# Gadersd/stable-diffusion-burn

Measured on NVIDIA H100. Metric: images_per_sec_512x512_20steps, higher is better.
Workload: dtype fp16 tensor-core operands (3-term split-fp16 on the two high-res UNet levels), fp32 accumulate

## Files before the change

stable_diffusion_burn_b200/csrc/api.cu:

```cuda
#include "../../include/sdb200.h"

#include <dlfcn.h>

#include <cstdlib>
#include <cstring>
#include <mutex>

#include "attention.cuh"
#include "kernels.cuh"
#include "model.cuh"
#include "runtime.cuh"

using namespace sdb;

struct sdb_ctx {
  Ctx c;
};

static thread_local std::string g_err;

#define API_BEGIN(ctxp)                      \
  if (!(ctxp)) {                             \
    g_err = "null context";                  \
    return 1;                                \
// ... 305 lines not shown
  API_BEGIN(ctx)
  need_final(c);
  model_sample_dev(c, d_context, n, L, d_uncond, Lu, guidance_scale, n_steps, d_init_latent, H, W, nullptr, d_rgb,
                   (cudaStream_t)stream);
  API_END
}

int sdb_forward_diffuser(sdb_ctx* ctx, const float* latent, int32_t timestep, const float* context, int n, int L,
                         const float* uncond, int Lu, double guidance_scale, int H, int W, float* pred, float* out_uncond,
                         float* out_cond) {
  API_BEGIN(ctx)
  need_final(c);
  SDB_CHECK(latent && context && uncond, "null argument");
  model_forward_diffuser_host(c, latent, timestep, context, n, L, uncond, Lu, guidance_scale, H, W, pred, out_uncond, out_cond);
  API_END
}

int sdb_forward_diffuser_dev(sdb_ctx* ctx, const float* d_latent, int32_t timestep, const float* d_context, int n, int L,
                             const float* d_uncond, int Lu, double guidance_scale, int H, int W, float* d_pred, void* stream) {
  API_BEGIN(ctx)
  need_final(c);
  model_forward_diffuser_dev(c, d_latent, timestep, d_context, n, L, d_uncond, Lu, guidance_scale, H, W, d_pred, nullptr, nullptr,
                             (cudaStream_t)stream);
  API_END
}

int sdb_encode_image(sdb_ctx* ctx, const float* img, int n, int H, int W, float* latent) {
  API_BEGIN(ctx)
  need_final(c);
  SDB_CHECK(img && latent, "null argument");
  model_encode_host(c, img, n, H, W, latent);
  API_END
}

int sdb_encode_image_dev(sdb_ctx* ctx, const float* d_img, int n, int H, int W, float* d_latent, void* stream) {
  API_BEGIN(ctx)
  need_final(c);
  model_encode_dev(c, d_img, n, H, W, d_latent, (cudaStream_t)stream);
  API_END
}

int sdb_clip_forward(sdb_ctx* ctx, const int32_t* tokens, int n, int L, float* out) {
  API_BEGIN(ctx)
  need_final(c);
  SDB_CHECK(tokens && out, "null argument");
  model_clip_forward_host(c, tokens, n, L, out);
  API_END
}

int sdb_clip_forward_dev(sdb_ctx* ctx, const int32_t* d_tokens, int n, int L, float* d_out, void* stream) {
  API_BEGIN(ctx)
  need_final(c);
  model_clip_forward_dev(c, d_tokens, n, L, d_out, (cudaStream_t)stream);
  API_END
}

int sdb_set_option(sdb_ctx* ctx, const char* key, int value) {
  API_BEGIN(ctx)
  const std::string k = key ? key : "";
  if (k == "precision")
    c.opt_precision = value;
  else if (k == "graphs")
    c.opt_graphs = value;
  else if (k == "splitk")
    c.opt_splitk = value;
  else if (k == "raw16")
    c.opt_raw16 = value;
  else if (k == "splitk_min_iters")
    c.opt_splitk_min_iters = value;
  else if (k == "splitk_chunk")
    c.opt_splitk_chunk = value < 1 ? 1 : value;
  else if (k == "attn_split")
    c.opt_attn_split = value;
  else if (k == "attn_regsplit")
    g_attn_regsplit = value;
  else if (k == "emb_hoist")
    c.opt_emb_hoist = value;
  else if (k == "prefetch_w")
    c.opt_prefetch_w = value;
  else if (k == "mlp_passes")
    c.opt_mlp_passes = value;
  else if (k == "gn_epilogue")
    c.opt_gn_epilogue = value;
  else if (k == "skip_merge")
    c.opt_skip_merge = value;
  else if (k == "gn_apply_ctas")
    g_gn_apply_ctas = value < 1 ? 1 : value;
  else if (k == "gn_min_pix")
    g_gn_min_pix = value < 1 ? 1 : value;
  else
    throw Error("unknown option: " + k);
  model_invalidate_graphs(c);
  API_END
}

int sdb_profile_enable(sdb_ctx* ctx, int on) {
  API_BEGIN(ctx)
  profile_collect(c);
  c.profiling = on != 0;
  API_END
}
int sdb_profile_reset(sdb_ctx* ctx) {
  API_BEGIN(ctx)
  profile_collect(c);
  c.launches = 0;
  for (int i = 0; i < KC_COUNT; ++i) c.cls_ms[i] = c.cls_flops[i] = c.cls_bytes[i] = c.cls_issued[i] = 0, c.cls_launches[i] = 0;
  API_END
}
int sdb_profile_class_count(sdb_ctx*) { return KC_COUNT; }
int sdb_profile_get(sdb_ctx* ctx, int cls, const char** name, int64_t* launches, double* ms, double* flops, double* bytes) {
  API_BEGIN(ctx)
  SDB_CHECK(cls >= 0 && cls < KC_COUNT, "class index");
  profile_collect(c);
  if (name) *name = kernel_class_name(cls);
  if (launches) *launches = c.cls_launches[cls];
  if (ms) *ms = c.cls_ms[cls];
  if (flops) *flops = c.cls_flops[cls];
  if (bytes) *bytes = c.cls_bytes[cls];
  API_END
}
int sdb_profile_get_issued(sdb_ctx* ctx, int cls, double* issued_flops) {
  API_BEGIN(ctx)
  SDB_CHECK(cls >= 0 && cls < KC_COUNT && issued_flops, "class index");
  *issued_flops = c.cls_issued[cls];
  API_END
}
int64_t sdb_launch_count(sdb_ctx* ctx) { return ctx ? ctx->c.launches : -1; }

int sdb_test_linear(sdb_ctx* ctx, const float* a, const float* w, const float* bias, int M, int K, int N, int passes,
                    float* out) {
  API_BEGIN(ctx)
  c.work.reset();
  float* d_a = c.work.get<float>((size_t)M * K);
  float* d_w = c.work.get<float>((size_t)K * N);
  float* d_b = bias ? c.work.get<float>(N) : nullptr;
  float* d_c = c.work.get<float>((size_t)M * N);
  SDB_CUDA(cudaMemcpyAsync(d_a, a, sizeof(float) * M * K, cudaMemcpyHostToDevice, c.stream));
  SDB_CUDA(cudaMemcpyAsync(d_w, w, sizeof(float) * K * N, cudaMemcpyHostToDevice, c.stream));
  if (bias) SDB_CUDA(cudaMemcpyAsync(d_b, bias, sizeof(float) * N, cudaMemcpyHostToDevice, c.stream));
  ActOp A;
  A.p.hi = c.work.get<__half>((size_t)M * K);
  A.p.lo = c.work.get<__half>((size_t)M * K);
  A.W = M, A.C = K;
  WeightOp Wp;
  Wp.p.hi = c.work.get<__half>((size_t)N * K);
  Wp.p.lo = c.work.get<__half>((size_t)N * K);
  Wp.N = N, Wp.K = K;
  convert_f16_launch(d_a, (long long)M * K, A.p, c.stream);
  pack_linear_launch(d_w, K, N, Wp.p, 0, c.stream);
  Epilogue ep;
  ep.out_f32 = d_c;
  ep.bias = d_b;
  run_gemm(c, G_LINEAR, A, nullptr, Wp, passes, ep);
  SDB_CUDA(cudaMemcpyAsync(out, d_c, sizeof(float) * M * N, cudaMemcpyDeviceToHost, c.stream));
  SDB_CUDA(cudaStreamSynchronize(c.stream));
  API_END
}

int sdb_test_gemm_ex(sdb_ctx* ctx, const float* a, const float* w, const float* bias, const float* residual, int M, int K, int N,
                     int passes, int flags, const float* xa, const float* xw, int XK, float* out) {
  API_BEGIN(ctx)
  c.work.reset();
  const bool geglu = flags & 1, from_f16 = flags & 4;
  SDB_CHECK(!geglu || (N % 128 == 0 && !residual && !xa), "GEGLU test: N (= 2 * hidden) must be a multiple of 128, no residual / extra K");
  const int Nout = geglu ? N / 2 : N;
  auto up = [&](const float* h, size_t cnt) {
// ... 319 lines not shown
```

stable_diffusion_burn_b200/csrc/gemm_tc.cu:

```cuda
#include "gemm_tc.cuh"

#include <cstring>

namespace sdb {

static constexpr int BM = 128;
static constexpr int BK = 64;
static constexpr int A_TILE_BYTES = BM * BK * 2;

template <int BN, int PASSES>
struct StageLayout {
  static constexpr int B_TILE_BYTES = BN * BK * 2;
  static constexpr int A_TILES = PASSES >= 2 ? 2 : 1;
  static constexpr int B_TILES = PASSES >= 3 ? 2 : 1;
  static constexpr int BYTES = A_TILES * A_TILE_BYTES + B_TILES * B_TILE_BYTES;
};
template <int BN>
struct AccLayout {
  static constexpr int PITCH = (BN + 4) * 4;
  static constexpr int BYTES = BM * PITCH;
  static constexpr int GN_BYTES = 32 * 1024;
};
static constexpr int EW = 8;

__device__ __noinline__ void epilogue_store(float4 f, unsigned int o32, unsigned int o16, float* out_f32, __half* out_f16,
                                            __half* out_f16_lo, int act) {
  if (act == 1) {
    f.x = __fdividef(f.x, 1.0f + __expf(-1.702f * f.x)), f.y = __fdividef(f.y, 1.0f + __expf(-1.702f * f.y));
    f.z = __fdividef(f.z, 1.0f + __expf(-1.702f * f.z)), f.w = __fdividef(f.w, 1.0f + __expf(-1.702f * f.w));
  }
  if (out_f32) *reinterpret_cast<float4*>(out_f32 + o32) = f;
  if (out_f16) {
    __half2 h[2] = {f2h2_sat(f.x, f.y), f2h2_sat(f.z, f.w)};
    *reinterpret_cast<uint2*>(out_f16 + o16) = *reinterpret_cast<uint2*>(h);
    if (out_f16_lo) {
      const float2 f0 = __half22float2(h[0]), f1 = __half22float2(h[1]);
      __half2 l[2] = {__floats2half2_rn(f.x - f0.x, f.y - f0.y), __floats2half2_rn(f.z - f1.x, f.w - f1.y)};
      *reinterpret_cast<uint2*>(out_f16_lo + o16) = *reinterpret_cast<uint2*>(l);
    }
  }
}

struct GnTile {
  int tn, img0, tile, nimg;
};
__device__ __forceinline__ GnTile gn_tile_of(const GemmParams& p, int n0, int th, int tw) {
  GnTile g;
  if (p.gn_rpi) {
    g.nimg = p.gn_nimg;
    if (p.gn_rpi >= BM)
      g.tn = 1, g.img0 = (tw * BM) / p.gn_rpi, g.tile = ((tw * BM) % p.gn_rpi) / BM;
    else
      g.tn = BM / p.gn_rpi, g.img0 = tw * g.tn, g.tile = 0;
  } else {
    g.tn = p.TN, g.img0 = n0, g.tile = th * p.tiles_w + tw, g.nimg = p.nimg;
  }
  return g;
}
__device__ __forceinline__ void gn_write_partials(const GemmParams& p, const float2* cs, int BN, int te, int nthreads, const GnTile g,
                                                  int col0, int z) {
  const int nbk_tile = BN / p.gn_bucket, nbk_total = p.N / p.gn_bucket;
  const int qpi = 4 / g.tn;
  const int slot = p.gn_slot0 + g.tile * p.split_k + z;
  (void)nthreads;
  if (te < ((nbk_tile * 4 + 31) & ~31)) {
    const int b = te >> 2, q = te & 3;
    float sm = 0.f, sq = 0.f;
    if (b < nbk_tile) {
      const float2* src = cs + q * BN + b * p.gn_bucket;
      for (int c = 0; c < p.gn_bucket; ++c) sm += src[c].x, sq += src[c].y;
    }
    if (qpi >= 2) sm += __shfl_xor_sync(0xffffffffu, sm, 1), sq += __shfl_xor_sync(0xffffffffu, sq, 1);
    if (qpi == 4) sm += __shfl_xor_sync(0xffffffffu, sm, 2), sq += __shfl_xor_sync(0xffffffffu, sq, 2);
    const int k = q / qpi, img = g.img0 + k, c0 = b * p.gn_bucket;
    if (b < nbk_tile && (q % qpi) == 0 && img < g.nimg && col0 + c0 < p.N) {
      float2* dst = reinterpret_cast<float2*>(p.gn_part) + ((size_t)img * p.gn_cap + slot) * nbk_total + (col0 + c0) / p.gn_bucket;
      *dst = make_float2(sm, sq);
    }
  }
}

enum : int { EPI_PLAIN = 0, EPI_GN = 1, EPI_LNS = 2, EPI_LNC = 3, EPI_GEGLU = 4, EPI_GEGLU_LNC = 5 };

template <int BN, int PASSES, int STAGES>
// ... 427 lines not shown
#pragma unroll
            for (int b4 = 0; b4 < 2; ++b4) {
              float4 t[4];
#pragma unroll
              for (int i = 0; i < 4; ++i)
                asm volatile("ld.shared.v4.f32 {%0, %1, %2, %3}, [%4];"
                             : "=f"(t[i].x), "=f"(t[i].y), "=f"(t[i].z), "=f"(t[i].w)
                             : "r"(tl + (b4 * 4 + i) * 4 * TROW)
                             : "memory");
#pragma unroll
              for (int i = 0; i < 4; ++i) {
                const int k = b4 * 4 + i;
                if (mr8[k] < 0) continue;
                float4 f = t[i];
                if constexpr (kLNC) {
                  f.x = rs8[k] * (f.x - mu8[k] * us[j].x), f.y = rs8[k] * (f.y - mu8[k] * us[j].y);
                  f.z = rs8[k] * (f.z - mu8[k] * us[j].z), f.w = rs8[k] * (f.w - mu8[k] * us[j].w);
                }
                if constexpr (kLNC)
                  f.x += bvs[j].x, f.y += bvs[j].y, f.z += bvs[j].z, f.w += bvs[j].w;
                else
                  f.x += bvs[j].x + ad[k].x, f.y += bvs[j].y + ad[k].y, f.z += bvs[j].z + ad[k].z, f.w += bvs[j].w + ad[k].w;
                if constexpr (kLNS) {
                  lrs[k] += (f.x + f.y) + (f.z + f.w);
                  lrq[k] = fmaf(f.x, f.x, fmaf(f.y, f.y, fmaf(f.z, f.z, fmaf(f.w, f.w, lrq[k]))));
                }
                if constexpr (kGN) {
                  gsum.x += f.x, gsum.y += f.y, gsum.z += f.z, gsum.w += f.w;
                  gsq.x = fmaf(f.x, f.x, gsq.x), gsq.y = fmaf(f.y, f.y, gsq.y), gsq.z = fmaf(f.z, f.z, gsq.z), gsq.w = fmaf(f.w, f.w, gsq.w);
                }
                epilogue_store(f, (unsigned)(mr8[k] * p.ldc + col), (unsigned)(mr8[k] * p.ldc16 + col), p.out_f32, p.out_f16,
                               p.out_f16_lo, p.act);
              }
            }
          }
          if constexpr (kGN) {
#pragma unroll
            for (int o = 8; o <= 16; o <<= 1) {
              gsum.x += __shfl_xor_sync(0xffffffffu, gsum.x, o), gsum.y += __shfl_xor_sync(0xffffffffu, gsum.y, o);
              gsum.z += __shfl_xor_sync(0xffffffffu, gsum.z, o), gsum.w += __shfl_xor_sync(0xffffffffu, gsum.w, o);
              gsq.x += __shfl_xor_sync(0xffffffffu, gsq.x, o), gsq.y += __shfl_xor_sync(0xffffffffu, gsq.y, o);
              gsq.z += __shfl_xor_sync(0xffffffffu, gsq.z, o), gsq.w += __shfl_xor_sync(0xffffffffu, gsq.w, o);
            }
            if (sub == 0) {
              float2* d = gn_cs + q * BN + c + cq;
              d[0] = make_float2(gsum.x, gsq.x), d[1] = make_float2(gsum.y, gsq.y);
              d[2] = make_float2(gsum.z, gsq.z), d[3] = make_float2(gsum.w, gsq.w);
            }
          }
          if (j + 1 < NCH && c + CSTEP < BN) issue_addends(col0 + c + CSTEP + cq);
        }
      }
      if constexpr (kLNS) {
#pragma unroll
        for (int k = 0; k < 8; ++k) {
#pragma unroll
          for (int o = 1; o <= 4; o <<= 1) {
            lrs[k] += __shfl_xor_sync(0xffffffffu, lrs[k], o);
            lrq[k] += __shfl_xor_sync(0xffffffffu, lrq[k], o);
          }
        }
        if ((lane & 7) == 0) {
          const int slot = blockIdx.y * 2 + half;
#pragma unroll
          for (int k = 0; k < 8; ++k)
            if (mr8[k] >= 0) {
              float2* d = reinterpret_cast<float2*>(p.ln_out) + (size_t)mr8[k] * p.ln_slots + slot;
              d[0] = make_float2(lrs[k], lrq[k]);
              if (EG == 1) d[1] = make_float2(0.f, 0.f);
            }
        }
      }
      if constexpr (kGN) {
        asm volatile("bar.sync 1, %0;" ::"n"(EW * 32) : "memory");
        gn_write_partials(p, gn_cs, BN, threadIdx.x - 128, EW * 32, gnt, col0, p.up2 ? (int)blockIdx.z * p.gn_phase_slots : 0);
      }
    }
    if (dbg && threadIdx.x == 128) dbg[6] = clock64();
  }
  __syncthreads();
  if (dbg && threadIdx.x == 0) dbg[7] = clock64();
}

static constexpr int SMEM_OPTIN_MAX = 227 * 1024;
template <int BN, int PASSES>
constexpr int pick_stages() {
  constexpr int per = StageLayout<BN, PASSES>::BYTES;
  constexpr int n = (SMEM_OPTIN_MAX - 1024) / (per + 2 * 8);
  return n > 8 ? 8 : n;
}

template <int BN, int PASSES, int STAGES, int EPI>
static void launch_epi(const GemmMaps& maps, const GemmParams& p, cudaStream_t stream) {
  constexpr int smem = region_bytes<BN, PASSES, STAGES>() + 2 * STAGES * 8 + 1024;
  static_assert(smem <= SMEM_OPTIN_MAX, "shared memory per block");
  static_assert(4 * BN * 8 <= AccLayout<BN>::GN_BYTES && 2 * (EW * 32) * 4 * 16 <= AccLayout<BN>::GN_BYTES,
                "GroupNorm column sums must fit in the scratch after the accumulator image");
  static DeviceOnce once;
  if (once.first())
    SDB_CUDA(cudaFuncSetAttribute(gemm_tc_kernel<BN, PASSES, STAGES, EPI>, cudaFuncAttributeMaxDynamicSharedMemorySize, smem));
  dim3 grid(p.tiles_n * p.tiles_h * p.tiles_w, (p.N + BN - 1) / BN, p.up2 ? 4 : p.split_k);
  launch_k(gemm_tc_kernel<BN, PASSES, STAGES, EPI>, grid, dim3(128 + 32 * EW), (size_t)smem, stream, maps, p);
}
template <int BN, int PASSES, int STAGES>
static void launch_inst(const GemmMaps& maps, const GemmParams& p, cudaStream_t stream) {
  SDB_CHECK((p.gn_part != nullptr) + (p.ln_out != nullptr) + (p.ln_in != nullptr) <= 1, "one statistics role per launch");
  if constexpr (BN == 128) {
    if (p.geglu) {
      SDB_CHECK(!p.gn_part && !p.ln_out && p.split_k == 1, "GEGLU epilogue: no statistics output, no split-K");
      return p.ln_in ? launch_epi<BN, PASSES, STAGES, EPI_GEGLU_LNC>(maps, p, stream)
                     : launch_epi<BN, PASSES, STAGES, EPI_GEGLU>(maps, p, stream);
    }
  }
  SDB_CHECK(!p.geglu, "the GEGLU epilogue is built for 128-wide tiles");
  if constexpr (BN >= 128) {
    if (p.gn_part) return launch_epi<BN, PASSES, STAGES, EPI_GN>(maps, p, stream);
  }
  if constexpr (BN == 160) {
    if (p.ln_out) return launch_epi<BN, PASSES, STAGES, EPI_LNS>(maps, p, stream);
  }
  if constexpr (BN == 128 || BN == 160) {
    if (p.ln_in) return launch_epi<BN, PASSES, STAGES, EPI_LNC>(maps, p, stream);
  }
  SDB_CHECK(!p.gn_part && !p.ln_out && !p.ln_in, "this statistics epilogue is not built for this tile width");
  launch_epi<BN, PASSES, STAGES, EPI_PLAIN>(maps, p, stream);
}
bool gemm_tc_supports(int BN, int epi) {
  return epi == EPI_PLAIN || (epi == EPI_GN && BN >= 128) || (epi == EPI_LNS && BN == 160) || (epi == EPI_LNC && (BN == 128 || BN == 160));
}

template <int BN, int PASSES>
static void launch_bn(const GemmMaps& maps, const GemmParams& p, cudaStream_t stream) {
  launch_inst<BN, PASSES, pick_stages<BN, PASSES>()>(maps, p, stream);
}

void gemm_tc_launch(const GemmMaps& maps, const GemmParams& p, int BN, int passes, cudaStream_t stream) {
  SDB_CHECK(p.TN * p.TH * p.TW == BM, "M tile must cover 128 rows");
  SDB_CHECK(p.N % 32 == 0, "N must be a multiple of 32");
#define SDB_DISPATCH(bn)                                             \
  case bn:                                                           \
    if (passes == 1) launch_bn<bn, 1>(maps, p, stream);              \
    else if (passes == 2) launch_bn<bn, 2>(maps, p, stream);         \
    else launch_bn<bn, 3>(maps, p, stream);                          \
    break;
  switch (BN) {
    SDB_DISPATCH(64)
    SDB_DISPATCH(128)
    SDB_DISPATCH(160)
    SDB_DISPATCH(256)
    default:
      throw Error("unsupported BN");
  }
#undef SDB_DISPATCH
}

}
```

stable_diffusion_burn_b200/csrc/gemm_tc.cuh:

```cuda
#pragma once
#include "common.cuh"

namespace sdb {

struct GemmMaps {
  CUtensorMap a[4][2];
  CUtensorMap bx[2];
  CUtensorMap b[2];
};

struct GemmParams {
  int nimg, H, W;
  int TN, TH, TW;
  int tiles_n, tiles_h, tiles_w;
  int N;
  int kc;
  int kc0;
  int num_taps;
  int xkc, xkc0;
  int8_t tap_dh[9], tap_dw[9], tap_ph[9];
  int split_k;
  int up2, gn_phase_slots;
  float* out_f32;
  __half* out_f16;
  __half* out_f16_lo;
  const float* bias;
  const float* rowbias;
  const float* residual;
  int ldc;
  int ldc16;
  int geglu;
  long long* dbg;
  int prefetch_w;
  int pdl_late;
  int act;
  float* gn_part;
  int gn_cap, gn_bucket, gn_slot0;
  int gn_rpi, gn_nimg;
  float* ln_out;
  int ln_slots;
  const float* ln_in;
  int ln_in_slots, ln_C;
  float ln_eps;
  const float* ln_u;
  const __half* res_hi;
  const __half* res_lo;
  float* ws;
  unsigned int* tickets;
  int OH, OW, os, oa, ob;
};

struct GemmLaunch {
  int BN, passes, stages;
};

void gemm_tc_launch(const GemmMaps& maps, const GemmParams& p, int BN, int passes, cudaStream_t stream);
bool gemm_tc_supports(int BN, int epi);
int gemm_tc_smem_bytes(int BN, int passes, int stages);

}
```

stable_diffusion_burn_b200/csrc/runtime.cu:

```cuda
#include "runtime.cuh"

#include <algorithm>

#include <cudaTypedefs.h>

#include <cmath>
#include <cstdlib>
#include <cstring>

namespace sdb {

int g_pdl_late = 1;
bool g_pdl_enabled = true;
int g_num_sms = 132;

void Arena::init(size_t bytes) {
  SDB_CUDA(cudaMalloc(&base, bytes));
  cap = bytes;
  off = 0;
}
void Arena::destroy() {
  if (base) cudaFree(base);
  base = nullptr;
  cap = off = 0;
// ... 225 lines not shown
  SDB_CHECK(passes < 2 || a0.p.lo, "multi-pass GEMM needs the lo half of A");
  SDB_CHECK(passes < 2 || !a1in || a1.p.lo, "multi-pass GEMM needs the lo half of A1");
  SDB_CHECK(passes < 3 || w.p.lo, "3-pass GEMM needs the lo half of W");

  GemmParams p;
  memset(&p, 0, sizeof(p));
  const int Ctot = a0.C + (a1in ? a1.C : 0);
  p.nimg = a0.n, p.H = a0.H, p.W = a0.W;
  p.N = w.N;
  p.kc = Ctot / 64;
  p.kc0 = a0.C / 64;
  int phases_out = 1;
  switch (kind) {
    case G_LINEAR:
      p.num_taps = 1;
      break;
    case G_CONV3:
      p.num_taps = 9;
      for (int t = 0; t < 9; ++t) p.tap_dh[t] = t / 3 - 1, p.tap_dw[t] = t % 3 - 1, p.tap_ph[t] = 0;
      break;
    case G_CONV3_S2:
      SDB_CHECK(a0.P == 4, "stride-2 conv needs a 4-phase operand");
      p.num_taps = 9;
      for (int t = 0; t < 9; ++t) {
        const int kh = t / 3, kw = t % 3;
        p.tap_dh[t] = kh == 0 ? -1 : 0;
        p.tap_dw[t] = kw == 0 ? -1 : 0;
        p.tap_ph[t] = (kh != 1 ? 2 : 0) + (kw != 1 ? 1 : 0);
      }
      break;
    case G_CONV3_S2_PAD01:
      SDB_CHECK(a0.P == 4, "stride-2 conv needs a 4-phase operand");
      p.num_taps = 9;
      for (int t = 0; t < 9; ++t) {
        const int kh = t / 3, kw = t % 3;
        p.tap_dh[t] = kh == 2 ? 1 : 0;
        p.tap_dw[t] = kw == 2 ? 1 : 0;
        p.tap_ph[t] = (kh == 1 ? 2 : 0) + (kw == 1 ? 1 : 0);
      }
      break;
    case G_CONV3_UP2:
      p.num_taps = 4;
      phases_out = 4;
      break;
    default:
      throw Error("bad gemm kind");
  }
  SDB_CHECK(w.K == p.num_taps * Ctot, "weight K does not match the operand");
  if (xk) {
    const int xC = xk->x0.C + (xk->has_x1 ? xk->x1.C : 0);
    SDB_CHECK(kind == G_CONV3 || kind == G_LINEAR, "extra-K operands need an unshifted output grid");
    SDB_CHECK(xk->x0.n == a0.n && xk->x0.H == a0.H && xk->x0.W == a0.W && xk->x0.P == 1 && xk->x0.C % 64 == 0, "extra-K geometry");
    SDB_CHECK(!xk->has_x1 || (xk->x1.n == a0.n && xk->x1.H == a0.H && xk->x1.W == a0.W && xk->x1.C % 64 == 0), "extra-K geometry");
    SDB_CHECK(xk->w.N == w.N && xk->w.K == xC, "extra-K weights");
    SDB_CHECK(passes < 2 || (xk->x0.p.lo && (!xk->has_x1 || xk->x1.p.lo)), "multi-pass GEMM needs the lo half of the extra operands");
    SDB_CHECK(passes < 3 || xk->w.p.lo, "3-pass GEMM needs the lo half of the extra weights");
    p.xkc0 = xk->x0.C / 64, p.xkc = xC / 64;
  }

  p.TW = std::min(pow2_floor(a0.W), 128);
  p.TH = std::min(128 / p.TW, pow2_ceil(a0.H));
  p.TN = 128 / (p.TW * p.TH);
  p.tiles_w = (a0.W + p.TW - 1) / p.TW;
  p.tiles_h = (a0.H + p.TH - 1) / p.TH;
  p.tiles_n = (a0.n + p.TN - 1) / p.TN;
  const int m_tiles = p.tiles_w * p.tiles_h * p.tiles_n;

  int BN;
  if (ep.geglu)
    BN = 128;
  else if (w.N % 160 == 0)
    BN = 160;
  else if (w.N % 256 == 0 && (long long)m_tiles * (w.N / 256) >= 2 * g_num_sms)
    BN = 256;
  else if (w.N % 128 == 0)
    BN = 128;
  else
    BN = 64;
  if (ep.ln_out) {
    SDB_CHECK(w.N % 160 == 0 && !ep.geglu, "LayerNorm statistics need an output width that tiles by 160");
    BN = 160;
  }
  if (ep.ln_in) SDB_CHECK(BN == 128 || BN == 160, "LayerNorm-consuming GEMM: tile width");
  const int n_tiles = (w.N + BN - 1) / BN;


  const int iters = p.num_taps * p.kc + p.xkc;
  int split = 1;
  if (c.opt_splitk && kind != G_CONV3_UP2 && !ep.geglu && !ep.ln_out && !ep.ln_in) {
    const int ctas = m_tiles * n_tiles;
    if (ctas <= g_num_sms / 2 && iters >= c.opt_splitk_min_iters) {
      split = std::min(std::min(g_num_sms / ctas, iters / c.opt_splitk_chunk), 16);
      if (split < 1) split = 1;
    }
  }
  if (split > 1) {
    const int per = (iters + split - 1) / split;
    split = (iters + per - 1) / per;
  }
  p.split_k = split;
  static const bool gemm_dbg = getenv("SDB_GEMM_DBG") != nullptr || getenv("SDB_LABEL_LOG") != nullptr;
  if (c.debug_sync || c.profiling || gemm_dbg) {
    char buf[256];
    snprintf(buf, sizeof(buf), "gemm kind=%d n=%d H=%d W=%d P=%d C0=%d C1=%d N=%d K=%d xk=%d BN=%d split=%d passes=%d geglu=%d epi=%s%s tile=%dx%dx%d",
             kind, a0.n, a0.H, a0.W, a0.P, a0.C, a1in ? a1.C : 0, w.N, w.K, p.xkc * 64, BN, split, passes, ep.geglu,
             ep.gn ? "gn" : (ep.ln_out ? "lns" : (ep.ln_in ? "lnc" : "-")), ep.residual16.hi ? "+r16" : (ep.residual ? "+r32" : ""), p.TN, p.TH, p.TW);
    c.dbg_label = buf;
  }

  GnPart* gn = ep.gn;
  if (gn) {
    int slots = m_tiles / p.tiles_n * split * phases_out;
    bool geom = p.TN <= 4;
    if (kind == G_LINEAR && gn_rpi > 0) {
      const long long rows = (long long)a0.W;
      geom = rows % gn_rpi == 0 && (gn_rpi % 128 == 0 || (128 % gn_rpi == 0 && gn_rpi >= 32));
      gn_nimg = (int)(rows / gn_rpi);
      slots = (gn_rpi >= 128 ? gn_rpi / 128 : 1) * split;
    } else {
      if (kind == G_LINEAR) geom = false;
      gn_rpi = 0;
    }
    const bool ok = gn->buf && gn->bucket > 0 && !ep.geglu && geom && BN >= 128 && BN % gn->bucket == 0 && w.N % gn->bucket == 0 &&
                    slots <= gn->cap && c.opt_gn_epilogue;
    gn->slots = ok ? slots : 0;
    if (!ok) gn = nullptr;
  }
  if (c.trace_on)
    c.gemm_trace.push_back({kind_in, w.N, BN, split, p.TN, p.TH, p.TW, p.xkc * 64, gn ? gn->slots : 0, a1in ? a1.C : 0});
  p.gn_part = gn ? gn->buf : nullptr;
  p.gn_cap = gn ? gn->cap : 0, p.gn_bucket = gn ? gn->bucket : 1;
  p.gn_rpi = gn ? gn_rpi : 0, p.gn_nimg = gn_nimg;
  p.ln_out = ep.ln_out, p.ln_slots = ln_slots(w.N);
  p.ln_in = ep.ln_in, p.ln_in_slots = ep.ln_in_slots, p.ln_C = ep.ln_C, p.ln_eps = ep.ln_eps;
  p.ln_u = passes >= 3 ? ep.ln_u_full : ep.ln_u_hi;
  SDB_CHECK(!ep.ln_in || (p.ln_u && ep.ln_in_slots > 0 && ep.ln_C == w.K && kind == G_LINEAR), "LayerNorm-consuming GEMM: arguments");
  SDB_CHECK(!ep.ln_in || (!ep.residual && !ep.rowbias && !ep.residual16.hi), "LayerNorm-consuming GEMM: no residual / row bias");
  SDB_CHECK(!ep.ln_out || kind == G_LINEAR, "LayerNorm statistics: rows must be tokens");
  p.res_hi = ep.residual16.hi, p.res_lo = ep.residual16.lo;
  SDB_CHECK(!ep.residual16.hi || (ep.residual16.lo && !ep.residual && !ep.rowbias), "fp16-pair residual: needs both halves, excludes the fp32 residual / row bias");
  p.out_f32 = ep.out_f32;
  p.out_f16 = ep.out_f16.hi;
  p.out_f16_lo = ep.out_f16.lo;
  p.bias = ep.bias;
  p.rowbias = ep.rowbias;
  p.residual = ep.residual;
  p.geglu = ep.geglu;
  p.act = ep.act;
  p.pdl_late = g_pdl_late;
  p.prefetch_w = (g_pdl_enabled && c.opt_prefetch_w && m_tiles <= 4) ? 1 : 0;
  const int nout = ep.geglu ? w.N / 2 : w.N;
  p.ldc = ep.ldc ? ep.ldc : nout;
  p.ldc16 = ep.ldc16 ? ep.ldc16 : nout;
  SDB_CHECK(!(ep.rowbias && ep.residual), "epilogue takes a time-embedding row or a residual, not both");
  p.os = (kind == G_CONV3_UP2) ? 2 : 1;
  p.OH = a0.H * p.os, p.OW = a0.W * p.os;
  SDB_CHECK((double)a0.n * p.OH * p.OW * (double)std::max(p.ldc, p.ldc16) < 2147483648.0,
            "GEMM output exceeds 2^31 elements (the epilogue uses 32-bit element offsets)");

  GemmMaps maps;
  memset(&maps, 0, sizeof(maps));
  maps.a[0][0] = make_act_map(a0.p.hi, a0.C, a0.W, a0.H, a0.P, a0.n, p.TW, p.TH, p.TN);
  maps.a[0][1] = maps.a[0][0];
  if (passes >= 2) maps.a[0][1] = make_act_map(a0.p.lo, a0.C, a0.W, a0.H, a0.P, a0.n, p.TW, p.TH, p.TN);
  maps.a[1][0] = maps.a[0][0];
  maps.a[1][1] = maps.a[0][1];
  if (a1in) {
    SDB_CHECK(a1.n == a0.n && a1.H == a0.H && a1.W == a0.W && a1.P == a0.P, "concat operand geometry");
    maps.a[1][0] = make_act_map(a1.p.hi, a1.C, a1.W, a1.H, a1.P, a1.n, p.TW, p.TH, p.TN);
    maps.a[1][1] = maps.a[1][0];
    if (passes >= 2) maps.a[1][1] = make_act_map(a1.p.lo, a1.C, a1.W, a1.H, a1.P, a1.n, p.TW, p.TH, p.TN);
  }

  for (int sidx = 2; sidx < 4; ++sidx) maps.a[sidx][0] = maps.a[sidx][1] = maps.a[0][0];
  if (xk) {
    auto xmaps = [&](const ActOp& x, int sidx) {
      maps.a[sidx][0] = make_act_map(x.p.hi, x.C, x.W, x.H, x.P, x.n, p.TW, p.TH, p.TN);
      maps.a[sidx][1] = passes >= 2 ? make_act_map(x.p.lo, x.C, x.W, x.H, x.P, x.n, p.TW, p.TH, p.TN) : maps.a[sidx][0];
    };
    xmaps(xk->x0, 2);
    if (xk->has_x1) xmaps(xk->x1, 3);
  }

  const double Mtot = (double)a0.n * a0.H * a0.W;
  const double flops = 2.0 * Mtot * (double)w.N * ((double)w.K + 64.0 * p.xkc);
  const double a_bytes = Mtot * (Ctot + 64.0 * p.xkc) * 2.0 * (passes >= 2 ? 2 : 1);
  const double w_bytes = (double)w.N * (w.K + 64.0 * p.xkc) * 2.0 * (passes >= 3 ? 2 : 1);
  const double o_bytes = Mtot * nout * ((ep.out_f32 ? 4.0 : 0.0) + (ep.out_f16.hi ? 2.0 : 0.0) + (ep.out_f16.lo ? 2.0 : 0.0)) +
                         (ep.residual ? Mtot * nout * 4.0 : 0.0);
  const double bytes = a_bytes + w_bytes + o_bytes;

  {
    const __half* whi = w.p.hi;
    const __half* wlo = w.p.lo;
    const int wrows = (w.rows ? w.rows : w.N) * phases_out;
    const int bbox = BN;
    maps.b[0] = make_w_map(whi, w.K, wrows, bbox, w.ld);
    maps.b[1] = maps.b[0];
    if (passes >= 3) maps.b[1] = make_w_map(wlo, w.K, wrows, bbox, w.ld);
    maps.bx[0] = maps.bx[1] = maps.b[0];
    if (xk) {
      const int xrows = xk->w.rows ? xk->w.rows : xk->w.N;
      maps.bx[0] = make_w_map(xk->w.p.hi, xk->w.K, xrows, bbox, xk->w.ld);
      maps.bx[1] = passes >= 3 ? make_w_map(xk->w.p.lo, xk->w.K, xrows, bbox, xk->w.ld) : maps.bx[0];
    }
    p.gn_slot0 = 0;
    p.up2 = 0, p.gn_phase_slots = (m_tiles / p.tiles_n) * split;
    if (kind == G_CONV3_UP2) {
      p.up2 = 1, p.oa = 0, p.ob = 0;
      for (int t = 0; t < 4; ++t) p.tap_dh[t] = (t >> 1) - 1, p.tap_dw[t] = (t & 1) - 1, p.tap_ph[t] = 0;
    }
    if (split > 1) {
      const size_t need = (size_t)split * (size_t)Mtot * w.N * sizeof(float);
      p.ws = reinterpret_cast<float*>(c.work.alloc(need));
      SDB_CHECK((long long)m_tiles * n_tiles * 2 <= 65536, "split-K ticket buffer");
      SDB_CHECK((long long)m_tiles * n_tiles * split <= g_num_sms, "split-K CTAs must be co-resident");
      p.tickets = c.splitk_tickets;
    }
    {
      static const bool dbg_on = getenv("SDB_GEMM_DBG") != nullptr;
      static long long* dbg_buf = nullptr;
      if (dbg_on) {
        if (!dbg_buf) SDB_CUDA(cudaMallocManaged(&dbg_buf, 16 * sizeof(long long)));
        SDB_CUDA(cudaStreamSynchronize(c.stream));
        memset(dbg_buf, 0, 16 * sizeof(long long));
        p.dbg = dbg_buf;
      }
      const std::string label = c.dbg_label;
      {
        KernelScope ks(c, KC_GEMM, flops * phases_out, bytes * phases_out, flops * passes * phases_out);
        gemm_tc_launch(maps, p, BN, passes, c.stream);
      }
      if (dbg_on) {
        SDB_CUDA(cudaStreamSynchronize(c.stream));
        fprintf(stderr, "gemm_dbg %s | cycles since entry: prologue %lld tma0 %lld landed %lld lastmma %lld accum %lld epi %lld exit %lld | chunk0: ld %lld stage %lld finish %lld (bias %lld loads0 %lld batch0 %lld)\n",
                label.c_str(), dbg_buf[1] - dbg_buf[0], dbg_buf[2] - dbg_buf[0], dbg_buf[3] - dbg_buf[0],
                dbg_buf[4] - dbg_buf[0], dbg_buf[5] - dbg_buf[0], dbg_buf[6] - dbg_buf[0], dbg_buf[7] - dbg_buf[0], dbg_buf[9] - dbg_buf[8], dbg_buf[10] - dbg_buf[9],
                dbg_buf[11] - dbg_buf[10], dbg_buf[12] - dbg_buf[10], dbg_buf[13] - dbg_buf[12], dbg_buf[14] - dbg_buf[13]);
      }
    }
  }
}

}
```

stable_diffusion_burn_b200/csrc/runtime.cuh:

```cuda
#pragma once
#include <string>
#include <unordered_map>
#include <unordered_set>
#include <vector>

#include "common.cuh"
#include "attention.cuh"
#include "gemm_tc.cuh"
#include "kernels.cuh"

namespace sdb {

struct Arena {
  char* base = nullptr;
  size_t cap = 0, off = 0, high = 0;
  void init(size_t bytes);
  void destroy();
  void* alloc(size_t bytes);
  template <class T>
  T* get(size_t count) {
    return reinterpret_cast<T*>(alloc(count * sizeof(T)));
  }
  void reset() { off = 0; }
};
// ... 17 lines not shown
  KC_ATTN,
  KC_GN_STATS,
  KC_PREP,
  KC_LAYERNORM,
  KC_SMALLCONV,
  KC_ELEMENTWISE,
  KC_COUNT
};

struct ProfEvent {
  int cls;
  cudaEvent_t a, b;
  double flops, bytes;
  std::string label;
};

struct ActOp {
  Half2Ptr p;
  int n = 1, P = 1, H = 1, W = 1, C = 0;
};
struct WeightOp {
  Half2Ptr p;
  int N = 0, K = 0;
  long long ld = 0;
  int rows = 0;
};
enum GemmKind : int { G_LINEAR = 0, G_CONV1 = 1, G_CONV3 = 2, G_CONV3_S2 = 3, G_CONV3_UP2 = 4, G_CONV3_S2_PAD01 = 5 };

struct GnPart {
  float* buf = nullptr;
  int cap = 0, bucket = 0, slots = 0;
};

struct Epilogue {
  float* ln_out = nullptr;
  const float* ln_in = nullptr;
  int ln_in_slots = 0, ln_C = 0;
  float ln_eps = 1e-5f;
  const float* ln_u_hi = nullptr;
  const float* ln_u_full = nullptr;
  Half2Ptr residual16;
  GnPart* gn = nullptr;
  int gn_rpi = 0;
  float* out_f32 = nullptr;
  Half2Ptr out_f16;
  const float* bias = nullptr;
  const float* rowbias = nullptr;
  const float* residual = nullptr;
  int geglu = 0;
  int act = 0;
  int ldc = 0;
  int ldc16 = 0;
};

struct MetaCheck {
  std::string relpath;
  std::vector<float> values;
  bool must_be_absent = false;
};

struct Ctx {
  int device = 0;
  cudaStream_t stream = nullptr;
  bool own_stream = true;
  std::string err;
  Arena master, packed, work;
  std::vector<TensorInfo> tensors;
  std::unordered_map<std::string, int> index;
  bool finalized = false;
  std::vector<MetaCheck> meta;
  std::unordered_set<std::string> group_norms;
  std::unordered_map<std::string, float> norm_eps;
  int opt_precision = 0;
  int opt_graphs = 1;
  int opt_splitk = 1;
  int opt_splitk_min_iters = 32, opt_splitk_chunk = 8;
  int opt_skip_merge = 1;
  int opt_raw16 = 1;
  int opt_mlp_passes = 0;
  int opt_attn_split = 1;
  int opt_emb_hoist = 1;
  int opt_prefetch_w = 0;
  int opt_gn_epilogue = 1;
  bool profiling = false;
  std::vector<ProfEvent> prof;
  int64_t launches = 0;
  double cls_ms[KC_COUNT] = {0}, cls_flops[KC_COUNT] = {0}, cls_bytes[KC_COUNT] = {0};
  double cls_issued[KC_COUNT] = {0};
  int64_t cls_launches[KC_COUNT] = {0};
  struct IoBuf {
    void* p = nullptr;
    size_t cap = 0;
  } iobuf[6];
  void* io(int slot, size_t bytes);
  void io_destroy();
  void* model = nullptr;
  unsigned int* splitk_tickets = nullptr;
  bool debug_sync = false;
  std::string dbg_label;
  struct GemmRecord {
    int kind, N, BN, split, TN, TH, TW, xk_channels, gn_slots, a1_channels;
  };
  bool trace_on = false;
  std::vector<GemmRecord> gemm_trace;
  std::vector<int> gn_trace;

  float* master_ptr(const std::string& name);
  const TensorInfo& info(const std::string& name);
  bool has(const std::string& name) const { return index.count(name) != 0; }
};

struct KernelScope {
  Ctx& c;
  int cls;
  bool on;
  ProfEvent ev;
  KernelScope(Ctx& c, int cls, double flops = 0, double bytes = 0, double issued = 0);
  ~KernelScope();
};
void profile_collect(Ctx& c);

struct ExtraK {
  ActOp x0, x1;
  bool has_x1 = false;
  WeightOp w;
};

void run_gemm(Ctx& c, int kind, const ActOp& a0, const ActOp* a1, const WeightOp& w, int passes, const Epilogue& ep,
              const ExtraK* xk = nullptr);

struct AttnOp {
  const __half* q = nullptr;
  int ldq = 0, q_col0 = 0, q_rows = 0;
  const __half* k = nullptr;
  int ldk = 0, k_col0 = 0, k_rows = 0;
  const __half* q_lo = nullptr;
  const __half* k_lo = nullptr;
  const __half* vT = nullptr;
  int ldv = 0;
  int v_mn = 0, v_col0 = 0;
  int nb = 1, heads = 8, d = 0, dpad = 0, Nq = 0, Nk = 0;
  const int* kvlen = nullptr;
  int causal = 0;
  Half2Ptr out;
  int ldo = 0;
};
void run_attention(Ctx& c, const AttnOp& a);
inline int ln_slots(int N) { return ((N + 159) / 160) * 2; }

const char* kernel_class_name(int cls);

}
```

Measured before the change: 5.028.

## Add persistent ping-pong warp-specialized GEMM for LayerNorm/GEGLU linear layers

Adds a persistent GEMM kernel with one TMA producer warpgroup and two consumer warpgroups that alternate output tiles. Each consumer's epilogue (LayerNorm-consume, GEGLU) overlaps the other's mainloop, and stores are staged through swizzled shared memory as coalesced 16-byte writes. It runs by default for multi-pass Linear GEMMs with GEGLU or LN-consuming epilogues when there are more tiles than SMs. The intent is to hide epilogue cost and tile-launch overhead. In exchange the tile width is fixed at 128, which may lower pipeline depth and adds a separate code path to maintain.

```diff
diff --git a/stable_diffusion_burn_b200/csrc/api.cu b/stable_diffusion_burn_b200/csrc/api.cu
--- a/stable_diffusion_burn_b200/csrc/api.cu
+++ b/stable_diffusion_burn_b200/csrc/api.cu
@@ -411,6 +411,8 @@
     c.opt_mlp_passes = value;
   else if (k == "gn_epilogue")
     c.opt_gn_epilogue = value;
+  else if (k == "gemm_persistent")
+    c.opt_gemm_persistent = value;
   else if (k == "skip_merge")
     c.opt_skip_merge = value;
   else if (k == "gn_apply_ctas")
diff --git a/stable_diffusion_burn_b200/csrc/gemm_tc.cu b/stable_diffusion_burn_b200/csrc/gemm_tc.cu
--- a/stable_diffusion_burn_b200/csrc/gemm_tc.cu
+++ b/stable_diffusion_burn_b200/csrc/gemm_tc.cu
@@ -1,5 +1,6 @@
 #include "gemm_tc.cuh"
 
+#include <algorithm>
 #include <cstring>
 
 namespace sdb {
@@ -593,6 +594,259 @@
   if (dbg && threadIdx.x == 0) dbg[7] = clock64();
 }
 
+static constexpr int PP_BN = 128;
+static constexpr int PP_STG_BYTES = 2 * 64 * 128;
+
+__device__ __forceinline__ uint32_t stg_off(int row, int col) {
+  return row * 128 + ((((col >> 3) ^ (row & 7)) << 4) | ((col & 7) * 2));
+}
+
+template <int PASSES, int STAGES, int EPI>
+__global__ void __launch_bounds__(384, 1)
+gemm_pp_kernel(const __grid_constant__ GemmMaps maps, const GemmParams p) {
+  constexpr int BN = PP_BN;
+  constexpr bool kLNC = EPI == EPI_LNC || EPI == EPI_GEGLU_LNC;
+  constexpr bool kGEGLU = EPI == EPI_GEGLU || EPI == EPI_GEGLU_LNC;
+  using L = StageLayout<BN, PASSES>;
+  extern __shared__ __align__(1024) uint8_t smem_raw[];
+  uint8_t* smem = smem_raw + ((1024u - (smem_u32(smem_raw) & 1023u)) & 1023u);
+  uint8_t* const stg_base = smem + STAGES * L::BYTES;
+  uint64_t* full_bar = reinterpret_cast<uint64_t*>(stg_base + 2 * PP_STG_BYTES);
+  uint64_t* empty_bar = full_bar + STAGES;
+
+  const int warp = threadIdx.x >> 5;
+  const int lane = threadIdx.x & 31;
+  if (!p.pdl_late) pdl_trigger();
+
+  const int m_tiles = p.tiles_n * p.tiles_h * p.tiles_w;
+  const int tiles = m_tiles * (p.N / BN);
+  const int my_tiles = (tiles - (int)blockIdx.x + (int)gridDim.x - 1) / (int)gridDim.x;
+  const int KC = p.kc;
+  auto tile_of = [&](int i, int& w0, int& h0, int& n0, int& col0) {
+    const int t = (int)blockIdx.x + i * (int)gridDim.x;
+    int mt = t % m_tiles;
+    col0 = (t / m_tiles) * BN;
+    const int tw = mt % p.tiles_w;
+    mt /= p.tiles_w;
+    w0 = tw * p.TW, h0 = (mt % p.tiles_h) * p.TH, n0 = (mt / p.tiles_h) * p.TN;
+  };
+
+  if (threadIdx.x == 0) {
+    for (int s = 0; s < STAGES; ++s) {
+      mbar_init(&full_bar[s], 1);
+      mbar_init(&empty_bar[s], 4);
+    }
+    fence_mbar_init();
+  }
+  __syncthreads();
+
+  if (warp < 4) {
+    asm volatile("setmaxnreg.dec.sync.aligned.u32 40;");
+    if (warp == 0 && elect_one()) {
+      tma_prefetch_desc(&maps.a[0][0]);
+      tma_prefetch_desc(&maps.b[0]);
+      if (p.kc0 < p.kc) tma_prefetch_desc(&maps.a[1][0]);
+      auto load_b = [&](int g, int s) {
+        int w0, h0, n0, col0;
+        tile_of(g / KC, w0, h0, n0, col0);
+        const int bk = (g % KC) * BK;
+        uint8_t* sb = smem + s * L::BYTES + L::A_TILES * A_TILE_BYTES;
+        tma_load_2d(sb, &maps.b[0], &full_bar[s], bk, col0);
+        if (PASSES >= 3) tma_load_2d(sb + L::B_TILE_BYTES, &maps.b[1], &full_bar[s], bk, col0);
+      };
+      auto load_a = [&](int g, int s) {
+        int w0, h0, n0, col0;
+        tile_of(g / KC, w0, h0, n0, col0);
+        const int cc = g % KC;
+        const int src = cc >= p.kc0 ? 1 : 0;
+        const int c0 = (cc - (src ? p.kc0 : 0)) * BK;
+        uint8_t* st = smem + s * L::BYTES;
+        tma_load_5d(st, &maps.a[src][0], &full_bar[s], c0, w0, h0, 0, n0);
+        if (PASSES >= 2) tma_load_5d(st + A_TILE_BYTES, &maps.a[src][1], &full_bar[s], c0, w0, h0, 0, n0);
+      };
+      const int total = my_tiles * KC;
+      const int npre = min(STAGES, total);
+      for (int g = 0; g < npre; ++g) {
+        mbar_expect_tx(&full_bar[g], L::BYTES);
+        load_b(g, g);
+      }
+      pdl_wait();
+      for (int g = 0; g < npre; ++g) load_a(g, g);
+      for (int g = npre; g < total; ++g) {
+        const int s = g % STAGES;
+        mbar_wait(&empty_bar[s], ((g / STAGES) & 1) ^ 1);
+        mbar_expect_tx(&full_bar[s], L::BYTES);
+        load_a(g, s);
+        load_b(g, s);
+      }
+    }
+  } else {
+    asm volatile("setmaxnreg.inc.sync.aligned.u32 232;");
+    pdl_wait();
+    const int wg = (warp - 4) >> 2;
+    const int w4 = warp & 3;
+    for (int i = wg; i < my_tiles; i += 2) {
+      int w0, h0, n0, col0;
+      tile_of(i, w0, h0, n0, col0);
+      auto row_m = [&](int r) {
+        const int pw = w0 + r % p.TW, ph = h0 + (r / p.TW) % p.TH, pn = n0 + r / (p.TW * p.TH);
+        return (pw < p.W && ph < p.H && pn < p.nimg) ? (pn * p.OH + ph) * p.OW + pw : -1;
+      };
+      float rmu[4] = {0.f, 0.f, 0.f, 0.f}, rrs[4] = {0.f, 0.f, 0.f, 0.f};
+      if constexpr (kLNC) {
+        const float2* sp[4];
+        float sm[4], sq[4];
+#pragma unroll
+        for (int e = 0; e < 4; ++e) {
+          const int m = row_m(64 * (e >> 1) + 16 * w4 + (lane >> 2) + 8 * (e & 1));
+          sp[e] = reinterpret_cast<const float2*>(p.ln_in) + (size_t)(m >= 0 ? m : 0) * p.ln_in_slots;
+          sm[e] = 0.f, sq[e] = 0.f;
+        }
+#pragma unroll 4
+        for (int k = 0; k < p.ln_in_slots; ++k) {
+          float2 v[4];
+#pragma unroll
+          for (int e = 0; e < 4; ++e) v[e] = sp[e][k];
+#pragma unroll
+          for (int e = 0; e < 4; ++e) sm[e] += v[e].x, sq[e] += v[e].y;
+        }
+        const float inv = 1.0f / (float)p.ln_C;
+#pragma unroll
+        for (int e = 0; e < 4; ++e) {
+          rmu[e] = sm[e] * inv;
+          rrs[e] = rsqrtf(fmaxf(sq[e] * inv - rmu[e] * rmu[e], 0.f) + p.ln_eps);
+        }
+      }
+      if (i > 0) {
+        if (wg == 0)
+          asm volatile("bar.sync 2, 256;" ::: "memory");
+        else
+          asm volatile("bar.sync 3, 256;" ::: "memory");
+      }
+      float acc[2][BN / 2];
+#pragma unroll
+      for (int h = 0; h < 2; ++h)
+#pragma unroll
+        for (int j = 0; j < BN / 2; ++j) acc[h][j] = 0.f;
+      int prev = -1;
+      for (int kk = 0; kk < KC; ++kk) {
+        const int g = i * KC + kk;
+        const int s = g % STAGES;
+        mbar_wait(&full_bar[s], (g / STAGES) & 1);
+        const uint32_t a_hi = smem_u32(smem + s * L::BYTES);
+        const uint32_t a_lo = a_hi + A_TILE_BYTES;
+        const uint32_t b_hi = a_hi + L::A_TILES * A_TILE_BYTES;
+        const uint32_t b_lo = b_hi + L::B_TILE_BYTES;
+        wgmma_fence();
+#pragma unroll
+        for (int k = 0; k < BK / 16; ++k) {
+          const uint32_t koff = k * 32;
+          const uint64_t db = make_sdesc_sw128(b_hi + koff);
+#pragma unroll
+          for (int h = 0; h < 2; ++h) {
+            const uint32_t ah = a_hi + h * (64 * 128) + koff;
+            const uint64_t da = make_sdesc_sw128(ah);
+            Wgmma<BN>::template ss<0>(acc[h], da, db, 1);
+            if (PASSES >= 2) Wgmma<BN>::template ss<0>(acc[h], make_sdesc_sw128(a_lo + h * (64 * 128) + koff), db, 1);
+            if (PASSES >= 3) Wgmma<BN>::template ss<0>(acc[h], da, make_sdesc_sw128(b_lo + koff), 1);
+          }
+        }
+        wgmma_commit();
+        wgmma_wait<1>();
+        if (prev >= 0 && lane == 0) mbar_arrive(&empty_bar[prev]);
+        prev = s;
+      }
+      if (i + 1 < my_tiles) {
+        if (wg == 0)
+          asm volatile("bar.arrive 3, 256;" ::: "memory");
+        else
+          asm volatile("bar.arrive 2, 256;" ::: "memory");
+      }
+
+      wgmma_wait<0>();
+      reg_fence(acc[0]);
+      reg_fence(acc[1]);
+      if (lane == 0) mbar_arrive(&empty_bar[prev]);
+      if (p.pdl_late && i + 2 >= my_tiles) pdl_trigger();
+
+      const int cq = 2 * (lane & 3);
+      uint8_t* const stg = stg_base + wg * PP_STG_BYTES;
+      auto stage = [&](int hh, int c, float x, float y) {
+        const uint32_t o = stg_off(16 * w4 + (lane >> 2) + 8 * hh, c);
+        const __half2 hv = f2h2_sat(x, y);
+        *reinterpret_cast<__half2*>(stg + o) = hv;
+        if (p.out_f16_lo) {
+          const float2 f = __half22float2(hv);
+          *reinterpret_cast<__half2*>(stg + PP_STG_BYTES / 2 + o) = __floats2half2_rn(x - f.x, y - f.y);
+        }
+      };
+      auto flush = [&](int h, int ocol) {
+        asm volatile("bar.sync %0, 128;" ::"r"(4 + wg) : "memory");
+        const int tl = threadIdx.x & 127, ch = tl & 7;
+#pragma unroll
+        for (int k = 0; k < 4; ++k) {
+          const int rl = (tl >> 3) + 16 * k;
+          const int m = row_m(64 * h + rl);
+          if (m >= 0) {
+            const uint32_t o = rl * 128 + ((ch ^ (rl & 7)) << 4);
+            const unsigned g = (unsigned)(m * p.ldc16 + ocol + ch * 8);
+            *reinterpret_cast<uint4*>(p.out_f16 + g) = *reinterpret_cast<const uint4*>(stg + o);
+            if (p.out_f16_lo) *reinterpret_cast<uint4*>(p.out_f16_lo + g) = *reinterpret_cast<const uint4*>(stg + PP_STG_BYTES / 2 + o);
+          }
+        }
+        asm volatile("bar.sync %0, 128;" ::"r"(4 + wg) : "memory");
+      };
+#pragma unroll
+      for (int h = 0; h < 2; ++h) {
+        if constexpr (kGEGLU) {
+          constexpr int HB = BN / 2;
+#pragma unroll
+          for (int jc = 0; jc < HB / 8; ++jc) {
+            const int c = 8 * jc + cq;
+            const float2 bx = *reinterpret_cast<const float2*>(p.bias + col0 + c);
+            const float2 bg = *reinterpret_cast<const float2*>(p.bias + col0 + HB + c);
+            float2 ux = make_float2(0.f, 0.f), ug = ux;
+            if constexpr (kLNC) {
+              ux = *reinterpret_cast<const float2*>(p.ln_u + col0 + c);
+              ug = *reinterpret_cast<const float2*>(p.ln_u + col0 + HB + c);
+            }
+#pragma unroll
+            for (int hh = 0; hh < 2; ++hh) {
+              const int e = 2 * h + hh, jx = 4 * jc + 2 * hh, jg = jx + HB / 2;
+              float2 tx = make_float2(acc[h][jx], acc[h][jx + 1]);
+              float2 tg = make_float2(acc[h][jg], acc[h][jg + 1]);
+              if constexpr (kLNC) {
+                tx.x = rrs[e] * (tx.x - rmu[e] * ux.x), tx.y = rrs[e] * (tx.y - rmu[e] * ux.y);
+                tg.x = rrs[e] * (tg.x - rmu[e] * ug.x), tg.y = rrs[e] * (tg.y - rmu[e] * ug.y);
+              }
+              stage(hh, c, (tx.x + bx.x) * gelu_erf_fast(tg.x + bg.x), (tx.y + bx.y) * gelu_erf_fast(tg.y + bg.y));
+            }
+          }
+          flush(h, col0 / 2);
+        } else {
+#pragma unroll
+          for (int half = 0; half < 2; ++half) {
+#pragma unroll
+            for (int jq = 0; jq < 8; ++jq) {
+              const int jc = 8 * half + jq, col = col0 + 8 * jc + cq;
+              const float2 u = *reinterpret_cast<const float2*>(p.ln_u + col);
+              const float2 b = p.bias ? *reinterpret_cast<const float2*>(p.bias + col) : make_float2(0.f, 0.f);
+#pragma unroll
+              for (int hh = 0; hh < 2; ++hh) {
+                const int e = 2 * h + hh, j = 4 * jc + 2 * hh;
+                float fx = rrs[e] * (acc[h][j] - rmu[e] * u.x), fy = rrs[e] * (acc[h][j + 1] - rmu[e] * u.y);
+                fx += b.x, fy += b.y;
+                stage(hh, 8 * jq + cq, fx, fy);
+              }
+            }
+            flush(h, col0 + 64 * half);
+          }
+        }
+      }
+    }
+  }
+}
+
 static constexpr int SMEM_OPTIN_MAX = 227 * 1024;
 template <int BN, int PASSES>
 constexpr int pick_stages() {
@@ -665,4 +919,40 @@
 #undef SDB_DISPATCH
 }
 
-}
+template <int PASSES>
+constexpr int pp_stages() {
+  constexpr int per = StageLayout<PP_BN, PASSES>::BYTES;
+  constexpr int n = (SMEM_OPTIN_MAX - 1024 - 2 * PP_STG_BYTES) / (per + 2 * 8);
+  return n > 8 ? 8 : n;
+}
+
+template <int PASSES, int EPI>
+static void launch_pp(const GemmMaps& maps, const GemmParams& p, cudaStream_t stream) {
+  constexpr int STAGES = pp_stages<PASSES>();
+  constexpr int smem = STAGES * StageLayout<PP_BN, PASSES>::BYTES + 2 * PP_STG_BYTES + 2 * STAGES * 8 + 1024;
+  static_assert(smem <= SMEM_OPTIN_MAX, "shared memory per block");
+  static DeviceOnce once;
+  if (once.first())
+    SDB_CUDA(cudaFuncSetAttribute(gemm_pp_kernel<PASSES, STAGES, EPI>, cudaFuncAttributeMaxDynamicSharedMemorySize, smem));
+  const int tiles = p.tiles_n * p.tiles_h * p.tiles_w * (p.N / PP_BN);
+  launch_k(gemm_pp_kernel<PASSES, STAGES, EPI>, dim3(std::min(tiles, g_num_sms)), dim3(384), (size_t)smem, stream, maps, p);
+}
+template <int PASSES>
+static void launch_pp_epi(const GemmMaps& maps, const GemmParams& p, cudaStream_t stream) {
+  if (!p.geglu) return launch_pp<PASSES, EPI_LNC>(maps, p, stream);
+  if (p.ln_in) return launch_pp<PASSES, EPI_GEGLU_LNC>(maps, p, stream);
+  launch_pp<PASSES, EPI_GEGLU>(maps, p, stream);
+}
+
+void gemm_tc_launch_persistent(const GemmMaps& maps, const GemmParams& p, int passes, cudaStream_t stream) {
+  SDB_CHECK(p.N % PP_BN == 0 && p.num_taps == 1 && p.xkc == 0 && p.split_k == 1 && !p.up2, "persistent GEMM: Linear, 128-wide N tiles");
+  SDB_CHECK(p.geglu || p.ln_in, "persistent GEMM: GEGLU or LayerNorm-consuming epilogue");
+  SDB_CHECK(p.ldc16 % 8 == 0, "persistent GEMM: 16-byte aligned fp16 output rows");
+  SDB_CHECK(!p.out_f32 && p.out_f16 && !p.act && !p.gn_part && !p.ln_out && !p.residual && !p.res_hi && !p.rowbias,
+            "persistent GEMM: fp16 output, no statistics output, residual or activation");
+  SDB_CHECK(passes == 2 || passes == 3, "persistent GEMM: 2- or 3-pass products");
+  if (passes == 2) launch_pp_epi<2>(maps, p, stream);
+  else launch_pp_epi<3>(maps, p, stream);
+}
+
+}
diff --git a/stable_diffusion_burn_b200/csrc/gemm_tc.cuh b/stable_diffusion_burn_b200/csrc/gemm_tc.cuh
--- a/stable_diffusion_burn_b200/csrc/gemm_tc.cuh
+++ b/stable_diffusion_burn_b200/csrc/gemm_tc.cuh
@@ -55,6 +55,7 @@
 };
 
 void gemm_tc_launch(const GemmMaps& maps, const GemmParams& p, int BN, int passes, cudaStream_t stream);
+void gemm_tc_launch_persistent(const GemmMaps& maps, const GemmParams& p, int passes, cudaStream_t stream);
 bool gemm_tc_supports(int BN, int epi);
 int gemm_tc_smem_bytes(int BN, int passes, int stages);
 
diff --git a/stable_diffusion_burn_b200/csrc/runtime.cu b/stable_diffusion_burn_b200/csrc/runtime.cu
--- a/stable_diffusion_burn_b200/csrc/runtime.cu
+++ b/stable_diffusion_burn_b200/csrc/runtime.cu
@@ -331,6 +331,11 @@
     BN = 160;
   }
   if (ep.ln_in) SDB_CHECK(BN == 128 || BN == 160, "LayerNorm-consuming GEMM: tile width");
+  const bool persistent = c.opt_gemm_persistent && kind == G_LINEAR && passes >= 2 && (ep.geglu || ep.ln_in) && !ep.gn && !ep.ln_out &&
+                          !ep.residual && !ep.residual16.hi && !ep.rowbias && !ep.out_f32 && ep.out_f16.hi && !ep.act && !xk &&
+                          w.N % 128 == 0 && (ep.ldc16 ? ep.ldc16 : w.N) % 8 == 0 &&
+                          (long long)m_tiles * (w.N / 128) > g_num_sms;
+  if (persistent) BN = 128;
   const int n_tiles = (w.N + BN - 1) / BN;
 
 
@@ -351,9 +356,10 @@
   static const bool gemm_dbg = getenv("SDB_GEMM_DBG") != nullptr || getenv("SDB_LABEL_LOG") != nullptr;
   if (c.debug_sync || c.profiling || gemm_dbg) {
     char buf[256];
-    snprintf(buf, sizeof(buf), "gemm kind=%d n=%d H=%d W=%d P=%d C0=%d C1=%d N=%d K=%d xk=%d BN=%d split=%d passes=%d geglu=%d epi=%s%s tile=%dx%dx%d",
+    snprintf(buf, sizeof(buf), "gemm kind=%d n=%d H=%d W=%d P=%d C0=%d C1=%d N=%d K=%d xk=%d BN=%d split=%d passes=%d geglu=%d epi=%s%s tile=%dx%dx%d persistent=%d",
              kind, a0.n, a0.H, a0.W, a0.P, a0.C, a1in ? a1.C : 0, w.N, w.K, p.xkc * 64, BN, split, passes, ep.geglu,
-             ep.gn ? "gn" : (ep.ln_out ? "lns" : (ep.ln_in ? "lnc" : "-")), ep.residual16.hi ? "+r16" : (ep.residual ? "+r32" : ""), p.TN, p.TH, p.TW);
+             ep.gn ? "gn" : (ep.ln_out ? "lns" : (ep.ln_in ? "lnc" : "-")), ep.residual16.hi ? "+r16" : (ep.residual ? "+r32" : ""), p.TN, p.TH, p.TW,
+             persistent ? 1 : 0);
     c.dbg_label = buf;
   }
 
@@ -478,7 +484,10 @@
       const std::string label = c.dbg_label;
       {
         KernelScope ks(c, KC_GEMM, flops * phases_out, bytes * phases_out, flops * passes * phases_out);
-        gemm_tc_launch(maps, p, BN, passes, c.stream);
+        if (persistent)
+          gemm_tc_launch_persistent(maps, p, passes, c.stream);
+        else
+          gemm_tc_launch(maps, p, BN, passes, c.stream);
       }
       if (dbg_on) {
         SDB_CUDA(cudaStreamSynchronize(c.stream));
diff --git a/stable_diffusion_burn_b200/csrc/runtime.cuh b/stable_diffusion_burn_b200/csrc/runtime.cuh
--- a/stable_diffusion_burn_b200/csrc/runtime.cuh
+++ b/stable_diffusion_burn_b200/csrc/runtime.cuh
@@ -123,6 +123,7 @@
   int opt_emb_hoist = 1;
   int opt_prefetch_w = 0;
   int opt_gn_epilogue = 1;
+  int opt_gemm_persistent = 1;
   bool profiling = false;
   std::vector<ProfEvent> prof;
   int64_t launches = 0;
```

New measurement: 5.112, median of 6. 1.02x the previous value.
